# atenpas/agile_grasp

Measured on AMD Instinct MI355X. Metric: grasp hypotheses/sec on 300k-pt cloud @2000 samples, higher is better.
Workload: dtype f64

## Files before the change

agile_grasp_amd/binding.py:

```python
from __future__ import annotations

import ctypes as C
import os

import numpy as np

_HERE = os.path.dirname(os.path.abspath(__file__))
_LIB = None

NORMALS_DETERMINISTIC = 0
NORMALS_RAND50 = 1


class AghParams(C.Structure):
    _fields_ = [
        ("finger_width", C.c_double),
        ("hand_outer_diameter", C.c_double),
        ("hand_depth", C.c_double),
        ("hand_height", C.c_double),
        ("init_bite", C.c_double),
        ("nn_radius_taubin", C.c_double),
        ("nn_radius_hands", C.c_double),
        ("nn_radius_normals", C.c_double),
        ("cam_origin", (C.c_double * 3) * 2),
# ... 21 lines not shown
        ("cam_source", "<i4"),
        ("n_in_box", "<i4"),
        ("half_antipodal", "u1"),
        ("full_antipodal", "u1"),
        ("svm_keep", "u1"),
        ("valid", "u1"),
        ("finger_index", "<i4"),
        ("depth_index", "<i4"),
        ("epoch", "<i4"),
    ]
)
FRAME_DTYPE = np.dtype(
    [
        ("sample", "<f8", 3),
        ("normal", "<f8", 3),
        ("axis", "<f8", 3),
        ("binormal", "<f8", 3),
        ("params", "<f8", 10),
        ("eigenvalue", "<f8"),
        ("n_nb", "<i4"),
        ("majority_cam", "<i4"),
        ("max_index", "<i4"),
        ("valid", "<i4"),
    ]
)
HANDLE_DTYPE = np.dtype([("axis", "<f8", 3), ("center", "<f8", 3), ("approach", "<f8", 3), ("binormal", "<f8", 3),
                         ("hands_center", "<f8", 3), ("width", "<f8"), ("n_inliers", "<i4"), ("first_inlier", "<i4")])
assert HYP_DTYPE.itemsize == 160 and FRAME_DTYPE.itemsize == 200 and HANDLE_DTYPE.itemsize == 136

EXPORTS = [
    "agh_default_params", "agh_create", "agh_destroy", "agh_last_error", "agh_set_cloud", "agh_set_cloud_device", "agh_set_cloud_batch", "agh_set_cloud_batch_device",
    "agh_preprocess", "agh_preprocess_device", "agh_localize", "agh_localize_device", "agh_localize_begin", "agh_localize_stage", "agh_localize_end", "agh_get_cloud", "agh_find_handles", "agh_find_hands", "agh_find_hands_device", "agh_load_svm", "agh_load_svm_file", "agh_classify",
    "agh_classify_device", "agh_get_frames", "agh_get_neighbor_counts", "agh_get_images", "agh_get_hog",
    "agh_get_normals", "agh_get_timing", "agh_get_timing_counts", "agh_set_profile", "agh_synchronize", "agh_selftest_math",
    "agh_set_training_images", "agh_get_training_images", "agh_hog_images", "agh_train_svm", "agh_save_svm_file",
    "agh_load_svm_model", "agh_get_learning_points", "agh_get_epoch", "agh_get_packed_images", "agh_classify_images", "agh_comm_rccl_origin",
    "agh_save_svm_file_ex", "agh_comm_unique_id", "agh_comm_init", "agh_comm_init_local", "agh_comm_destroy", "agh_comm_rank", "agh_comm_last_count", "agh_comm_last_exchange", "agh_comm_set_segment_records", "agh_comm_inject_fault",
    "agh_shard_slice", "agh_find_hands_sharded_device", "agh_find_hands_sharded", "agh_classify_sharded_device",
    "agh_classify_sharded", "agh_default_plane_params", "agh_remove_plane", "agh_get_plane_inliers",
    "agh_get_plane_candidates", "agh_plane_replay",
]


def comm_unique_id() -> bytes:
    buf = (C.c_uint8 * 128)()
    rc = load_library().agh_comm_unique_id(buf)
    if rc != 0:
        raise AghError(rc, "agh_comm_unique_id failed (is RCCL installed?)")
    return bytes(buf)


def comm_init_local(contexts) -> None:
    arr = (C.c_void_p * len(contexts))(*[c._h for c in contexts])
    rc = load_library().agh_comm_init_local(arr, C.c_int32(len(contexts)))
    if rc != 0:
        raise AghError(rc, "agh_comm_init_local failed")


def shard_slice(n: int, rank: int, n_ranks: int):
    lo, hi = C.c_int64(0), C.c_int64(0)
    load_library().agh_shard_slice(C.c_int64(n), C.c_int32(rank), C.c_int32(n_ranks), C.byref(lo), C.byref(hi))
    return lo.value, hi.value


def comm_rccl_origin() -> str:
    lib = load_library()
    lib.agh_comm_rccl_origin.restype = C.c_char_p
# ... 498 lines not shown
        return out[:n].copy(), keep[:n].copy()

    def find_hands_sharded_torch(self, samples_t, out_t, nout_t, calculates_antipodal: bool = False, stream=None):
        S = samples_t.shape[0]
        cap = out_t.numel() // 160
        r, g = self.comm_rank()
        lo, hi = shard_slice(S, r, g)
        self.last_samples = hi - lo
        self._check(self.lib.agh_find_hands_sharded_device(
            self._h, C.c_void_p(samples_t.data_ptr()), C.c_int64(S), C.c_int(1 if calculates_antipodal else 0),
            C.c_void_p(out_t.data_ptr()), C.c_int64(cap), C.c_void_p(nout_t.data_ptr()),
            C.c_void_p(stream) if stream else None))

    def classify_sharded_torch(self, keep_t=None, stream=None):
        self._check(self.lib.agh_classify_sharded_device(
            self._h, C.c_void_p(keep_t.data_ptr()) if keep_t is not None else None, C.c_void_p(stream) if stream else None))

    def hog(self):
        desc = np.zeros((max(self.last_n, 1), 3528), np.float32)
        sums = np.zeros(max(self.last_n, 1), np.float64)
        n = self._check(self.lib.agh_get_hog(self._h, _p(desc, C.c_float), _p(sums, C.c_double), C.c_int64(self.last_n)))
        return desc[:n], sums[:n]

    def timing(self, counts: bool = False):
        t = AghTiming()
        self._check(self.lib.agh_get_timing(self._h, C.byref(t)))
        ms = {t.name[i].decode(): float(t.ms[i]) for i in range(t.n)}
        if counts:
            cnt = (C.c_int32 * 16)()
            self._check(self.lib.agh_get_timing_counts(self._h, cnt, C.c_int32(16)))
            return ms, {t.name[i].decode(): int(cnt[i]) for i in range(t.n)}
        return ms

    def set_profile(self, level: int):
        self._check(self.lib.agh_set_profile(self._h, C.c_int32(level)))

    def synchronize(self):
        self._check(self.lib.agh_synchronize(self._h))

    def selftest_math(self, n: int = 1 << 20, seed: int = 1) -> int:
        return int(self.lib.agh_selftest_math(self._h, C.c_int64(n), C.c_uint64(seed)))

    def set_cloud_torch(self, xyz_t, cam_t, stream=None):
        assert xyz_t.is_cuda and xyz_t.is_contiguous()
        self._keep = [xyz_t, cam_t]
        self.n = xyz_t.shape[0]
        self._check(self.lib.agh_set_cloud_device(
            self._h, C.c_void_p(xyz_t.data_ptr()), C.c_int64(xyz_t.stride(0) * 4),
            C.c_void_p(cam_t.data_ptr()) if cam_t is not None else None, C.c_int64(self.n),
            C.c_void_p(stream) if stream else None))

    def find_hands_torch(self, samples_t, out_t, nout_t, calculates_antipodal: bool = False, stream=None):
        S = samples_t.shape[0]
        cap = out_t.numel() // 160
        self.last_samples = S
        self._check(self.lib.agh_find_hands_device(
            self._h, C.c_void_p(samples_t.data_ptr()), C.c_int64(S), C.c_int(1 if calculates_antipodal else 0),
            C.c_void_p(out_t.data_ptr()), C.c_int64(cap), C.c_void_p(nout_t.data_ptr()),
            C.c_void_p(stream) if stream else None))

    def classify_torch(self, keep_t=None, stream=None):
        self._check(self.lib.agh_classify_device(self._h, C.c_void_p(keep_t.data_ptr()) if keep_t is not None else None,
                                                 C.c_void_p(stream) if stream else None))
```

agile_grasp_amd/csrc/agh_internal.h:

```cpp
#pragma once

#include <hip/hip_runtime.h>
#include <stdint.h>

#include <string>
#include <vector>

#include "agh.h"

namespace agh
{

constexpr int kBboxBlocks = 128;
constexpr int kCellCap = 1 << 21;
constexpr int kCellStride = kCellCap + 4;
constexpr int kMaxRows = 128;
constexpr int kNumSums = 37;
constexpr int kSumStride = 40;
constexpr int kSlots = 8;
constexpr int kImageWords = 250;
constexpr int kBigListGrid = 512;
constexpr int kSweepWg4MinSamples = 4096;
constexpr int64_t kNormalsChunk = 16384;

struct GridDesc
{
  double mn[3];
  double cell;
  double inv_cell;
  int dim[3];
  int ncell;
  unsigned done;
  unsigned ticket;
};

constexpr int kMaxClouds = 64;
struct GridView
{
  const GridDesc* desc;
  const int* cell_start;
  const float4* sorted;
  const int* cloud_off;
  int n_clouds;
};

struct HandGeom
{
  double finger_width, hand_outer_diameter, hand_depth, hand_height, init_bite;
  double cam_origin[2][3];
  double cos_a[8], sin_a[8];
  double fs[20];
  double thr[40];
  int n_thr;
  int lo_idx[20], hi_idx[20];
  double depths[16];
  double backs[16];
  double boxy[16];
  int n_depths;
  double cos_antipodal;
  double xlut_lo, xlut_scale;
  double ylut_lo, ylut_scale;
  unsigned char xlut[1024];
  unsigned char ylut[64];
  int x_probes, y_probes;
};
// ... 110 lines not shown
  float* d_vox_xyz = nullptr;
  int32_t* d_vox_cam = nullptr;
  int64_t vox_cap = 0;
  float* d_raw_xyz = nullptr;
  float* d_stage_xyz = nullptr;
  int64_t stage_cap = 0;
  hipStream_t stage_stream = nullptr;
  hipEvent_t stage_done = nullptr;
  LocalizeState loc;
  int64_t raw_cap = 0;
  PlaneState* plane = nullptr;

  agh_hypothesis* d_h_hands = nullptr;
  unsigned long long* d_h_bits = nullptr;
  int* d_h_rowcnt = nullptr;
  int* d_h_first = nullptr;
  int* d_h_n = nullptr;
  int* d_h_idx = nullptr;
  int* d_h_counts = nullptr;
  int* d_h_tmp = nullptr;
  agh_handle* d_h_handles = nullptr;
  int64_t h_cap = 0;

  int n_clouds = 1;
  int clouds_cap = 0;
  std::vector<int64_t> cloud_off;
  std::vector<int32_t> cloud_off_i32;
  bool cloud_off_on_device = false;
  bool defer_cloud_count = false;
  bool n_is_bound = false;
  int* d_cloud_off = nullptr;
  int32_t* d_scloud = nullptr;
  GridDesc* d_desc = nullptr;
  float* d_bbox_part = nullptr;
  int* d_cell_start = nullptr;
  int* d_cell_count = nullptr;
  int* d_block_sums = nullptr;
  unsigned long long* d_tile_state = nullptr;
  unsigned build_gen = 0;
  bool grid_clean = false;
  int* d_cell_of = nullptr;
  int* d_rank_of = nullptr;
  float4* d_sorted = nullptr;
  int64_t grid_cap = 0;
  bool has_cloud = false;
  const int32_t* pending_cam_host = nullptr;
  int64_t pending_cam_n = 0;
  bool cloud_async = false;

  int64_t s_cap = 0;
  int32_t* d_samples = nullptr;
  double* d_sums = nullptr;
  int32_t* d_nt = nullptr;
  int32_t* d_ovf = nullptr;
  int32_t* d_nh = nullptr;
  int32_t* d_status = nullptr;
  int* d_weight = nullptr;
  uint8_t* d_vmask = nullptr;
  int* d_order = nullptr;
  int* d_order_sweep = nullptr;
  int order_frame_s = 0;
  const int32_t* order_frame_samples = nullptr;
  int order_sweep_s = 0;
  const int32_t* order_sweep_samples = nullptr;
  float4* d_nbr = nullptr;
  int64_t nbr_stride = 0;
  double* d_eig = nullptr;
// ... 278 lines not shown
{
  int begin[kMaxRows];
  int prefix[kMaxRows + 1];
  int seg_row[64];
  int nrows;
  int total;
  int bad;
};

constexpr double kSlabMargin = 1e-6;
template <bool SLAB = false>
__device__ __forceinline__ void build_rows(const GridView& gv, float qx, float qy, float qz, double rpad, RowTable& rt,
  const double* slab_axis = nullptr, double slab_hh = 0.0, const GridDesc* gpre = nullptr)
{
  const GridDesc& g = gpre ? *gpre : *gv.desc;
  const int tid = threadIdx.x;
  const int lx = cell_coord(g, (double) qx - rpad, 0), hx = cell_coord(g, (double) qx + rpad, 0);
  const int ly = cell_coord(g, (double) qy - rpad, 1), hy = cell_coord(g, (double) qy + rpad, 1);
  const int lz = cell_coord(g, (double) qz - rpad, 2), hz = cell_coord(g, (double) qz + rpad, 2);
  const int ny = hy - ly + 1, nz = hz - lz + 1;
  const int nrows = ny * nz;
  if (tid == 0)
  {
    rt.nrows = nrows;
    rt.bad = nrows > kMaxRows;
  }
  if (nrows <= kMaxRows)
  {
    for (int t = tid; t < nrows; t += blockDim.x)
    {
      const int tq = (int) (((float) t + 0.5f) * (1.0f / (float) ny));
      const int cy = ly + (t - tq * ny), cz = lz + tq;
      const double y0 = g.mn[1] + cy * g.cell, z0 = g.mn[2] + cz * g.cell;
      const double dy = fmax(fmax(y0 - (double) qy, (double) qy - (y0 + g.cell)), 0.0);
      const double dz = fmax(fmax(z0 - (double) qz, (double) qz - (z0 + g.cell)), 0.0);
      int b = 0, len = 0;
      const double rem = rpad * rpad - (dy * dy + dz * dz);
      if (rem >= 0.0)
      {
        const double xr = sqrt(rem);
        double xlo = (double) qx - xr, xhi = (double) qx + xr;
        bool keep = true;
        if (SLAB)
        {
          const double ya = (y0 - kSlabMargin) - (double) qy, yb = (y0 + g.cell + kSlabMargin) - (double) qy;
          const double za = (z0 - kSlabMargin) - (double) qz, zb = (z0 + g.cell + kSlabMargin) - (double) qz;
          const double ey0 = slab_axis[1] * ya, ey1 = slab_axis[1] * yb, ez0 = slab_axis[2] * za, ez1 = slab_axis[2] * zb;
          const double L = fmin(ey0, ey1) + fmin(ez0, ez1), U = fmax(ey0, ey1) + fmax(ez0, ez1);
          const double lo_n = (-1.0 * (slab_hh + kSlabMargin)) - U, hi_n = (slab_hh + kSlabMargin) - L;
          const double ax = slab_axis[0];
          if (fabs(ax) > 1e-9)
          {
            const double inv_ax = 1.0 / ax;
            const double b1 = lo_n * inv_ax, b2 = hi_n * inv_ax;
            xlo = fmax(xlo, ((double) qx + fmin(b1, b2)) - kSlabMargin);
            xhi = fmin(xhi, ((double) qx + fmax(b1, b2)) + kSlabMargin);
            keep = xlo <= xhi;
          }
          else
            keep = (lo_n < 0.0) & (hi_n > 0.0);
          keep = keep | !(L == L && U == U);
        }
        if (keep)
        {
          const int lxr = max(lx, cell_coord(g, xlo, 0)), hxr = min(hx, cell_coord(g, xhi, 0));
          const int base = (cz * g.dim[1] + cy) * g.dim[0];
          b = gv.cell_start[base + lxr];
          len = hxr >= lxr ? gv.cell_start[base + hxr + 1] - b : 0;
        }
      }
      rt.begin[t] = b;
      rt.prefix[t + 1] = len;
    }
  }
  __syncthreads();
  if (tid < 64)
// ... 197 lines not shown
```

agile_grasp_amd/csrc/api.hip:

```cpp
#include "agh_internal.h"

#include <algorithm>
#include <atomic>
#include <cmath>
#include <cstdio>
#include <cstdlib>
#include <cstring>

using namespace agh;


namespace
{
thread_local std::string g_create_error;
std::atomic<int32_t> g_epoch{ 0 };
}

namespace agh
{
int32_t next_epoch()
{
  int32_t e;
  do
    e = (int32_t) ((uint32_t) g_epoch.fetch_add(1) + 1u) & 0x7fffffff;
// ... 201 lines not shown
  return AGH_OK;
}

constexpr int64_t kMirrorMaxRecords = 1 << 16;
static inline int64_t pin_round(int64_t b) { return (b + 255) & ~(int64_t) 255; }
int ensure_host_staging(Ctx* c, int64_t samples, int64_t records)
{
  if (c->h_pin && samples <= c->h_pin_samples && records <= c->h_pin_records)
    return AGH_OK;
  const int64_t ns = std::max<int64_t>(std::max<int64_t>(samples, c->h_pin_samples), 1024);
  const int64_t nr = std::max<int64_t>(std::max<int64_t>(records, c->h_pin_records), 1024);
  if (c->h_pin)
  {
    HIPCHK(c, hipStreamSynchronize(c->stream));
    (void) hipHostFree(c->h_pin);
    c->h_pin = nullptr;
    c->h_pin_samples = c->h_pin_records = 0;
  }
  void* p = nullptr;
  HIPCHK(c, hipHostMalloc(&p, (size_t) (kPinHeaderBytes + pin_round(ns * 4) + nr * (int64_t) sizeof(agh_hypothesis)), hipHostMallocDefault));
  c->h_pin = static_cast<uint8_t*>(p);
  c->h_pin_samples = ns;
  c->h_pin_records = nr;
  return AGH_OK;
}

int ensure_clouds(Ctx* c, int C)
{
  if (C <= c->clouds_cap)
    return AGH_OK;
  int rc;
  if ((rc = dev_alloc(c, &c->d_desc, (size_t) C)) || (rc = dev_alloc(c, &c->d_cell_start, (size_t) C * (size_t) kCellStride)) ||
      (rc = dev_alloc(c, &c->d_cell_count, (size_t) C * kCellCap)) || (rc = dev_alloc(c, &c->d_bbox_part, (size_t) C * kBboxBlocks * 6)) ||
      (rc = dev_alloc(c, &c->d_tile_state, (size_t) C * (kCellCap / 1024))))
    return rc;
  c->clouds_cap = C;
  c->grid_clean = false;
  return AGH_OK;
}

int ensure_draws(Ctx* c, int64_t count, hipStream_t st)
{
  if (count <= c->draws_cap)
    return AGH_OK;
  std::vector<int32_t> h((size_t) count);
  GlibcRand g(c->p.rand_seed);
  for (int64_t i = 0; i < count; i++)
    h[i] = g.next();
  int rc;
  if ((rc = dev_alloc(c, &c->d_draws, (size_t) count)))
    return rc;
  HIPCHK(c, hipMemcpyAsync(c->d_draws, h.data(), sizeof(int32_t) * count, hipMemcpyHostToDevice, st));
  HIPCHK(c, hipStreamSynchronize(st));
  c->draws_cap = count;
  return AGH_OK;
}

__global__ void k_iota(int32_t* out, int base, int n)
{
  const int i = blockIdx.x * blockDim.x + threadIdx.x;
  if (i < n)
    out[i] = base + i;
}

int normals_pass(Ctx* c, int64_t p0, int64_t p1, hipStream_t st)
{
  for (int64_t b0 = p0; b0 < p1; b0 += kNormalsChunk)
// ... 107 lines not shown
  *out = nullptr;
  int ndev = 0;
  if (hipGetDeviceCount(&ndev) != hipSuccess || ndev <= 0)
  {
    g_create_error = "no HIP device is visible (this library has no CPU path)";
    return AGH_ERR_NO_DEVICE;
  }
  if (p->device < 0 || p->device >= ndev)
  {
    g_create_error = "device ordinal out of range";
    return AGH_ERR_INVALID_ARGUMENT;
  }
  hipDeviceProp_t prop;
  if (hipGetDeviceProperties(&prop, p->device) != hipSuccess)
  {
    g_create_error = "hipGetDeviceProperties failed";
    return AGH_ERR_HIP;
  }
  if (std::strncmp(prop.gcnArchName, "gfx950", 6) != 0)
  {
    g_create_error = std::string("device is ") + prop.gcnArchName + ", this build targets gfx950 (MI355X) only";
    return AGH_ERR_NO_DEVICE;
  }
  if (!(p->finger_width > 0) || !(p->hand_outer_diameter > p->finger_width) || !(p->hand_depth > 0) ||
      !(p->nn_radius_taubin > 0) || !(p->nn_radius_hands > 0) || !(p->nn_radius_normals > 0))
  {
    g_create_error = "invalid hand geometry or radii";
    return AGH_ERR_INVALID_ARGUMENT;
  }
  agh_ctx* ctx = new agh_ctx();
  Ctx* c = &ctx->c;
  c->p = *p;
  c->device = p->device;
#ifdef AGH_DEBUG_HOOKS
  if (const char* e = std::getenv("AGH_DEBUG_STOP_SWEEP"))
    c->debug_stop_sweep = std::atoi(e);
  if (const char* e = std::getenv("AGH_DEBUG_STOP_MOMENTS"))
    c->debug_stop_moments = std::atoi(e);
  if (const char* e = std::getenv("AGH_DEBUG_STOP_FRAME"))
    c->debug_stop_frame = std::atoi(e);
  if (const char* e = std::getenv("AGH_DEBUG_STOP_HOG"))
    c->debug_stop_hog = std::atoi(e);
#endif
  std::string gerr;
  build_geometry(*p, &c->geom, &gerr);
  if (!gerr.empty())
  {
    g_create_error = gerr;
    delete ctx;
    return AGH_ERR_INVALID_ARGUMENT;
  }
  auto fail = [&](int rc) {
    g_create_error = c->err;
    agh_destroy(ctx);
    return rc;
  };
  if (hipSetDevice(c->device) != hipSuccess || hipStreamCreate(&c->stream) != hipSuccess)
  {
    c->err = "hipSetDevice/hipStreamCreate failed";
    return fail(AGH_ERR_HIP);
  }
  int rc;
  if ((rc = ensure_clouds(c, 1)) || (rc = dev_alloc(c, &c->d_cloud_off, (size_t) kMaxClouds + 1)) ||
      (rc = dev_alloc(c, &c->d_block_sums, 4096)) ||
      (rc = dev_alloc(c, &c->d_flags, 8)) || (rc = dev_alloc(c, &c->d_nout, 1)) ||
      (rc = dev_alloc(c, &c->d_geom, 1)) || (rc = dev_alloc(c, &c->d_hog, 1)) ||
      (rc = dev_alloc(c, &c->d_svm_w, 3528)))
    return fail(rc);
  HogTablesDev* ht = new HogTablesDev();
  hog_tables_host(ht);
  hipError_t e1 = hipMemcpy(c->d_hog, ht, sizeof(HogTablesDev), hipMemcpyHostToDevice);
  delete ht;
  hipError_t e2 = hipMemcpy(c->d_geom, &c->geom, sizeof(HandGeom), hipMemcpyHostToDevice);
  hipError_t e3 = hipMemset(c->d_flags, 0, 8 * sizeof(int32_t));
  if (e1 != hipSuccess || e2 != hipSuccess || e3 != hipSuccess)
  {
    c->err = "uploading tables failed";
    return fail(AGH_ERR_HIP);
  }
  *out = ctx;
  return AGH_OK;
}

void agh_destroy(agh_ctx* ctx)
{
  if (!ctx)
    return;
  Ctx* c = &ctx->c;
  (void) hipSetDevice(c->device);
  if (c->stream)
    (void) hipStreamSynchronize(c->stream);
  comm_release(c);
  plane_release(c);
  void* ptrs[] = { c->own_xyz, c->own_cam, c->d_desc, c->d_bbox_part, c->d_cell_start, c->d_cell_count, c->d_block_sums, c->d_cell_of,
    c->d_rank_of, c->d_sorted, c->d_samples, c->d_sums, c->d_nt, c->d_nh, c->d_status, c->d_nbr, c->d_eig, c->d_frames, c->d_slots,
    c->d_images, c->d_slot_index, c->d_scan_tmp, c->d_out_own, c->d_nout, c->d_out_images, c->d_draw_ofs, c->d_draws,
    c->d_flags, c->d_normals, c->d_svm_w, c->d_hog, c->d_geom, c->d_desc_out, c->d_svm_sums, c->d_keep, c->d_vox_desc,
    c->d_weight, c->d_order, c->d_order_sweep, c->d_vmask, c->d_cloud_off, c->d_scloud, c->d_idx_own, c->d_tile_state, c->d_h_hands, c->d_h_bits, c->d_h_rowcnt, c->d_h_first,
    c->d_h_n, c->d_h_idx, c->d_h_counts, c->d_h_handles, c->d_h_tmp, c->d_images_cam, c->d_xbuf, c->d_nbuf, c->d_xcnt, c->d_cls_images, c->d_cls_keep, c->d_cls_sums, c->d_dbg, c->d_svm_svT, c->d_svm_alpha, c->d_cls_desc, c->d_cls_kbuf, c->d_vox_code, c->d_vox_blk, c->d_vox_blk2, c->d_vox_total, c->d_vox_bitmap, c->d_vox_xyz, c->d_vox_cam, c->d_raw_xyz, c->d_huge_stage, c->d_huge_key, c->d_huge_count, c->d_huge_sorted, c->d_huge_normals, c->d_huge_base, c->d_stage_xyz, c->d_ovf };
  for (void* p : ptrs)
    if (p)
      (void) hipFree(p);
  if (c->h_pin)
    (void) hipHostFree(c->h_pin);
  if (c->h_pin_handles)
    (void) hipHostFree(c->h_pin_handles);
  if (c->h_pin_keep)
    (void) hipHostFree(c->h_pin_keep);
  if (c->h_vox_desc)
    (void) hipHostFree(c->h_vox_desc);
  for (hipEvent_t e : c->ev)
    (void) hipEventDestroy(e);
  if (c->copy_done)
    (void) hipEventDestroy(c->copy_done);
  if (c->copy_gate)
    (void) hipEventDestroy(c->copy_gate);
  if (c->xyz_copied)
    (void) hipEventDestroy(c->xyz_copied);
  if (c->copy_stream)
    (void) hipStreamDestroy(c->copy_stream);
  if (c->stage_done)
    (void) hipEventDestroy(c->stage_done);
  if (c->stage_stream)
    (void) hipStreamDestroy(c->stage_stream);
  if (c->stream)
    (void) hipStreamDestroy(c->stream);
  delete ctx;
}

namespace
{
struct CloudOffArg
// ... 905 lines not shown
    float ms = 0.f;
    if (hipEventElapsedTime(&ms, c->ev[i - 1], c->ev[i]) != hipSuccess)
      ms = 0.f;
    int slot = -1;
    for (int j = 0; j < k; j++)
      if (std::strcmp(out->name[j], c->ev_name[i]) == 0)
        slot = j;
    if (slot < 0)
    {
      if (k >= AGH_TIMING_SLOTS)
        continue;
      slot = k++;
      out->name[slot] = c->ev_name[i];
    }
    out->ms[slot] += ms;
    c->timing_counts[slot]++;
    out->total_ms += ms;
  }
  out->n = k;
  c->ev_used = 0;
  c->ev_name.clear();
  return AGH_OK;
}

int agh_get_timing_counts(agh_ctx* ctx, int32_t* counts, int32_t cap)
{
  if (!ctx || !counts || cap < 0)
    return AGH_ERR_INVALID_ARGUMENT;
  for (int i = 0; i < cap && i < AGH_TIMING_SLOTS; i++)
    counts[i] = ctx->c.timing_counts[i];
  return AGH_OK;
}

int64_t agh_selftest_math(agh_ctx* ctx, int64_t n, uint64_t seed)
{
  if (!ctx)
    return AGH_ERR_INVALID_ARGUMENT;
  return selftest_math(&ctx->c, n, seed);
}

}
```

agile_grasp_amd/csrc/grid.hip:

```cpp
#include "agh_internal.h"

#include <algorithm>
#include <cstdlib>

namespace agh
{

__global__ void k_desc_reset(GridDesc* d)
{
  d += blockIdx.x;
  d->done = 0u;
  d->ticket = 0u;
}

__device__ void desc_finish(GridDesc* d, double base_cell, int64_t n, const float lo[3], const float hi[3])
{
  double mn[3], mx[3];
  for (int a = 0; a < 3; a++)
  {
    const bool any = n > 0 && lo[a] <= hi[a];
    mn[a] = any ? (double) lo[a] : 0.0;
    mx[a] = any ? (double) hi[a] : 0.0;
  }
  double cell = base_cell;
  int dim[3];
  for (;;)
  {
    double prod = 1.0;
    for (int a = 0; a < 3; a++)
    {
      dim[a] = (int) floor((mx[a] - mn[a]) / cell) + 1;
      prod *= (double) dim[a];
    }
    if (prod <= (double) kCellCap)
      break;
    cell *= 2.0;
  }
  for (int a = 0; a < 3; a++)
  {
    d->mn[a] = mn[a];
    d->dim[a] = dim[a];
  }
  d->cell = cell;
  d->inv_cell = 1.0 / cell;
// ... 20 lines not shown
      mn[a] = fminf(mn[a], fminf(pf ? pv[a] : INFINITY, qf ? qv[a] : INFINITY));
      mx[a] = fmaxf(mx[a], fmaxf(pf ? pv[a] : -INFINITY, qf ? qv[a] : -INFINITY));
    }
  }
  constexpr int kW = kBboxThreads / 64;
  __shared__ float smn[kW][3], smx[kW][3];
  for (int a = 0; a < 3; a++)
    for (int o = 32; o > 0; o >>= 1)
    {
      mn[a] = fminf(mn[a], __shfl_down(mn[a], o));
      mx[a] = fmaxf(mx[a], __shfl_down(mx[a], o));
    }
  if ((threadIdx.x & 63) == 0)
    for (int a = 0; a < 3; a++)
    {
      smn[threadIdx.x >> 6][a] = mn[a];
      smx[threadIdx.x >> 6][a] = mx[a];
    }
  __syncthreads();
  if (threadIdx.x < 3)
  {
    const int a = threadIdx.x;
    float lo = smn[0][a], hi = smx[0][a];
    for (int w = 1; w < kW; w++)
    {
      lo = fminf(lo, smn[w][a]);
      hi = fmaxf(hi, smx[w][a]);
    }
    part[blockIdx.x * 6 + a] = lo;
    part[blockIdx.x * 6 + 3 + a] = hi;
  }
}

__device__ __forceinline__ void desc_from_parts(const float* __restrict__ part, int nparts, double base_cell, int64_t n, GridDesc* g)
{
  __shared__ float red[4][6];
  const int tid = threadIdx.x, lane = tid & 63;
  float lo[3] = { INFINITY, INFINITY, INFINITY }, hi[3] = { -INFINITY, -INFINITY, -INFINITY };
  for (int b = tid; b < nparts; b += blockDim.x)
    for (int a = 0; a < 3; a++)
    {
      lo[a] = fminf(lo[a], part[b * 6 + a]);
      hi[a] = fmaxf(hi[a], part[b * 6 + 3 + a]);
    }
  for (int a = 0; a < 3; a++)
    for (int o = 32; o > 0; o >>= 1)
    {
      lo[a] = fminf(lo[a], __shfl_xor(lo[a], o));
      hi[a] = fmaxf(hi[a], __shfl_xor(hi[a], o));
    }
  if (lane == 0 && tid < 256)
    for (int a = 0; a < 3; a++)
    {
      red[tid >> 6][a] = lo[a];
      red[tid >> 6][3 + a] = hi[a];
    }
  __syncthreads();
  if (tid == 0)
  {
    for (int a = 0; a < 3; a++)
      for (int w = 1; w < 4; w++)
      {
        lo[a] = fminf(lo[a], red[w][a]);
        hi[a] = fmaxf(hi[a], red[w][3 + a]);
      }
    desc_finish(g, base_cell, n, lo, hi);
  }
  __syncthreads();
}

__global__ __launch_bounds__(256) void k_cell_count(const float* __restrict__ xyz, int64_t stride,
  const int* __restrict__ cloud_off, GridDesc* __restrict__ d, int* __restrict__ cell_of, int* __restrict__ rank_of,
  int* __restrict__ count, const float* __restrict__ part, int nparts, double base_cell)
{
  const int64_t p0 = cloud_off[blockIdx.y], n = cloud_off[blockIdx.y + 1] - p0;
  xyz += p0 * stride;
  cell_of += p0;
  rank_of += p0;
  count += (int64_t) blockIdx.y * kCellCap;
  __shared__ GridDesc gs;
  desc_from_parts(part + (int64_t) blockIdx.y * kBboxBlocks * 6, nparts, base_cell, n, &gs);
  const GridDesc g = gs;
  if (blockIdx.x == 0 && threadIdx.x == 0)
  {
    GridDesc* o = d + blockIdx.y;
    for (int a = 0; a < 3; a++)
    {
      o->mn[a] = g.mn[a];
      o->dim[a] = g.dim[a];
    }
    o->cell = g.cell;
    o->inv_cell = g.inv_cell;
    o->ncell = g.ncell;
  }
  const int lane = threadIdx.x & 63;
  const int64_t step = (int64_t) gridDim.x * blockDim.x;
  const int64_t n_up = (n + 63) & ~(int64_t) 63;
  for (int64_t i = blockIdx.x * (int64_t) blockDim.x + threadIdx.x; i < n_up; i += step)
  {
    int c = -1;
    if (i < n)
    {
      const float* p = xyz + i * stride;
      const int cx = cell_coord(g, (double) p[0], 0), cy = cell_coord(g, (double) p[1], 1),
                cz = cell_coord(g, (double) p[2], 2);
      c = (cz * g.dim[1] + cy) * g.dim[0] + cx;
      if (!(isfinite(p[0]) && isfinite(p[1]) && isfinite(p[2])))
        c = (int) (i % (int64_t) g.ncell);
    }
    const int prev = __shfl_up(c, 1);
    const bool head = (lane == 0) || (c != prev);
    const unsigned long long hm = __ballot(head);
    const int hl = 63 - __clzll((long long) (hm & ((2ull << lane) - 1ull)));
    const unsigned long long after = (hl == 63) ? 0ull : (hm >> (hl + 1));
    const int runlen = after ? (__ffsll((long long) after)) : (64 - hl);
    int base = 0;
    if (head && c >= 0)
      base = atomicAdd(&count[c], runlen);
    base = __shfl(base, hl);
    if (i < n)
    {
      cell_of[i] = c;
      rank_of[i] = base + (lane - hl);
    }
  }
}

constexpr int kScanBlock = 4096;

__device__ __forceinline__ int block_scan_excl(int v, int* total)
{
  __shared__ int wsum[4];
  const int lane = threadIdx.x & 63, w = threadIdx.x >> 6;
  const int inc = wave_incl_scan_i32(v);
  if (lane == 63)
    wsum[w] = inc;
  __syncthreads();
  int base = 0;
  for (int k = 0; k < w; k++)
    base += wsum[k];
  *total = wsum[0] + wsum[1] + wsum[2] + wsum[3];
  __syncthreads();
  return base + inc - v;
}

__global__ __launch_bounds__(256) void k_cell_scan(int* __restrict__ count, GridDesc* __restrict__ d,
  unsigned long long* __restrict__ tile_state, unsigned gen, int* __restrict__ cell_start, const int* __restrict__ cloud_off)
{
  __shared__ int s_prefix;
  const int p0 = cloud_off[blockIdx.y], n = cloud_off[blockIdx.y + 1] - p0;
  count += (int64_t) blockIdx.y * kCellCap;
  tile_state += (int64_t) blockIdx.y * (kCellCap / kScanBlock);
  cell_start += (int64_t) blockIdx.y * kCellStride;
  d += blockIdx.y;
  const int ncell = d->ncell;
  for (int tile = blockIdx.x; tile * kScanBlock < ncell; tile += gridDim.x)
  {
  const int b0 = tile * kScanBlock;
  int4 v[4];
  int sum = 0;
  for (int k = 0; k < 4; k++)
  {
    v[k] = reinterpret_cast<const int4*>(count + b0)[threadIdx.x * 4 + k];
    sum += (v[k].x + v[k].y) + (v[k].z + v[k].w);
  }
  int total;
  int ex = block_scan_excl(sum, &total);
  const unsigned long long tag = (unsigned long long) gen << 34;
  if (threadIdx.x < 64)
  {
    const int lane = threadIdx.x;
    int prefix = 0;
    if (lane == 0)
      __hip_atomic_store(&tile_state[tile], tag | ((tile == 0 ? 2ull : 1ull) << 32) | (unsigned) total, __ATOMIC_RELEASE,
        __HIP_MEMORY_SCOPE_AGENT);
    for (int j0 = tile - 1; j0 >= 0; j0 -= 64)
    {
      const int j = j0 - lane;
      unsigned long long w = 0;
      for (;;)
// ... 12 lines not shown
      const int stop = incl ? __ffsll((long long) incl) - 1 : 63;
      int val = (j >= 0 && lane <= stop) ? (int) (unsigned) w : 0;
      for (int o = 32; o > 0; o >>= 1)
        val += __shfl_xor(val, o);
      prefix += val;
      if (incl)
        break;
    }
    if (lane == 0)
    {
      if (tile != 0)
        __hip_atomic_store(&tile_state[tile], tag | (2ull << 32) | (unsigned) (prefix + total), __ATOMIC_RELEASE,
          __HIP_MEMORY_SCOPE_AGENT);
      s_prefix = prefix;
    }
  }
  __syncthreads();
  ex += s_prefix + p0;
  for (int k = 0; k < 4; k++)
  {
    int4 o;
    o.x = ex;
    o.y = o.x + v[k].x;
    o.z = o.y + v[k].y;
    o.w = o.z + v[k].z;
    ex = o.w + v[k].w;
    reinterpret_cast<int4*>(cell_start + b0)[threadIdx.x * 4 + k] = o;
    reinterpret_cast<int4*>(count + b0)[threadIdx.x * 4 + k] = make_int4(0, 0, 0, 0);
  }
  if (tile == 0 && threadIdx.x == 0)
    cell_start[ncell] = p0 + n;
  __syncthreads();
  }
}

__global__ __launch_bounds__(256) void k_scatter(const float* __restrict__ xyz, int64_t stride,
  const int32_t* __restrict__ cam, const int* __restrict__ cloud_off, const int* __restrict__ cell_of,
  const int* __restrict__ rank_of, const int* __restrict__ cell_start, float4* __restrict__ sorted)
{
  const int64_t p0 = cloud_off[blockIdx.y], p1 = cloud_off[blockIdx.y + 1];
  cell_start += (int64_t) blockIdx.y * kCellStride;
  for (int64_t i = p0 + blockIdx.x * (int64_t) blockDim.x + threadIdx.x; i < p1; i += (int64_t) gridDim.x * blockDim.x)
  {
    const int pos = cell_start[cell_of[i]] + rank_of[i];
    const float* p = xyz + i * stride;
    const unsigned w = ((unsigned) i << 1) | (cam ? (unsigned) (cam[i] & 1) : 0u);
    sorted[pos] = make_float4(p[0], p[1], p[2], __uint_as_float(w));
  }
}

int grid_build(Ctx* c, hipStream_t st)
{
  const int C = c->n_clouds;
  int64_t nmax = 0;
  for (int k = 0; k < C; k++)
    nmax = std::max<int64_t>(nmax, c->cloud_off[(size_t) k + 1] - c->cloud_off[(size_t) k]);
  const int nblk = (int) std::max<int64_t>(1, std::min<int64_t>((nmax + 255) / 256, 2048));
  if (!c->grid_clean)
  {
    hipMemsetAsync(c->d_cell_count, 0, sizeof(int) * (size_t) kCellCap * c->clouds_cap, st);
    hipMemsetAsync(c->d_tile_state, 0, sizeof(unsigned long long) * (size_t) (kCellCap / kScanBlock) * c->clouds_cap, st);
    hipLaunchKernelGGL(k_desc_reset, dim3(c->clouds_cap), dim3(1), 0, st, c->d_desc);
    c->build_gen = 0;
  }
  c->grid_clean = false;
  if (++c->build_gen >= (1u << 30))
  {
    hipMemsetAsync(c->d_tile_state, 0, sizeof(unsigned long long) * (size_t) (kCellCap / kScanBlock) * c->clouds_cap, st);
    c->build_gen = 1;
  }
  bool cam_gate = false;
  if (c->pending_cam_host)
  {
    if (!c->copy_stream && !c->copy_stream_failed &&
        (hipStreamCreateWithFlags(&c->copy_stream, hipStreamNonBlocking) != hipSuccess ||
         hipEventCreateWithFlags(&c->copy_done, hipEventDisableTiming) != hipSuccess ||
         hipEventCreateWithFlags(&c->copy_gate, hipEventDisableTiming) != hipSuccess))
    {
      if (c->copy_gate)
        (void) hipEventDestroy(c->copy_gate);
      if (c->copy_done)
        (void) hipEventDestroy(c->copy_done);
      if (c->copy_stream)
        (void) hipStreamDestroy(c->copy_stream);
      c->copy_gate = nullptr;
      c->copy_done = nullptr;
      c->copy_stream = nullptr;
      c->copy_stream_failed = true;
    }
    if (c->copy_stream)
      cam_gate = hipEventRecord(c->copy_gate, st) == hipSuccess && hipStreamWaitEvent(c->copy_stream, c->copy_gate, 0) == hipSuccess;
  }
  const double base_cell = std::max(0.02, c->p.nn_radius_hands / 4.0);
  const int nparts = std::max(1, std::min(nblk, kBboxBlocks));
  hipLaunchKernelGGL(k_bbox, dim3(nparts, C), dim3(kBboxThreads), 0, st, c->d_xyz, c->stride_floats,
    (const int*) c->d_cloud_off, c->d_bbox_part);
  hipLaunchKernelGGL(k_cell_count, dim3(nblk, C), dim3(256), 0, st, c->d_xyz, c->stride_floats, (const int*) c->d_cloud_off,
    c->d_desc, c->d_cell_of, c->d_rank_of, c->d_cell_count, (const float*) c->d_bbox_part, nparts, base_cell);
  hipLaunchKernelGGL(k_cell_scan, dim3(C == 1 ? 256 : 64, C), dim3(256), 0, st, c->d_cell_count, c->d_desc, c->d_tile_state,
    c->build_gen, c->d_cell_start, (const int*) c->d_cloud_off);
  if (c->pending_cam_host)
  {
    hipStream_t cs = (c->copy_stream && cam_gate) ? c->copy_stream : st;
    hipError_t e = hipMemcpyAsync(c->own_cam, c->pending_cam_host, sizeof(int32_t) * (size_t) c->pending_cam_n,
      hipMemcpyHostToDevice, cs);
    c->pending_cam_host = nullptr;
    c->cam_copy_on_copy_stream = cs != st;
    if (e == hipSuccess && cs != st)
    {
      e = hipEventRecord(c->copy_done, cs);
      if (e == hipSuccess)
        e = hipStreamWaitEvent(st, c->copy_done, 0);
    }
    if (e != hipSuccess)
      return AGH_ERR_HIP;
  }
  if (nmax > 0)
    hipLaunchKernelGGL(k_scatter, dim3(nblk, C), dim3(256), 0, st, c->d_xyz, c->stride_floats, c->d_cam,
      (const int*) c->d_cloud_off, c->d_cell_of, c->d_rank_of, c->d_cell_start, c->d_sorted);
  if (hipGetLastError() != hipSuccess)
    return AGH_ERR_HIP;
  c->grid_clean = true;
  return AGH_OK;
}

}
```

include/agh.h:

```cpp
#ifndef AGH_H
#define AGH_H

#include <stdint.h>

#ifdef __cplusplus
extern "C" {
#endif

#define AGH_VERSION 1

typedef enum agh_status
{
  AGH_OK = 0,
  AGH_ERR_INVALID_ARGUMENT = -1,
  AGH_ERR_NO_DEVICE = -2,
  AGH_ERR_HIP = -3,
  AGH_ERR_CAPACITY = -4,
  AGH_ERR_NO_CLOUD = -5,
  AGH_ERR_NO_SVM = -6,
  AGH_ERR_IO = -7,
  AGH_ERR_STATE = -8,
  AGH_ERR_RETRY = -9
} agh_status;

// ... 175 lines not shown
int agh_save_svm_file_ex(const char* path, int32_t kernel_type, const float* sv, int32_t n_sv, int32_t n_weights,
  const double* alpha, double rho, double C, int32_t max_iter, double eps);
int agh_load_svm_model(agh_ctx* ctx, int32_t kernel_type, const float* sv, int32_t n_sv, int32_t n_weights,
  const double* alpha, double rho);

#define AGH_COMM_ID_BYTES 128
int agh_comm_unique_id(uint8_t id[AGH_COMM_ID_BYTES]);
int agh_comm_init(agh_ctx* ctx, int32_t rank, int32_t n_ranks, const uint8_t id[AGH_COMM_ID_BYTES]);
int agh_comm_init_local(agh_ctx* const* ctxs, int32_t n_ranks);
int agh_comm_destroy(agh_ctx* ctx);
int agh_comm_rank(const agh_ctx* ctx, int32_t* rank, int32_t* n_ranks);
const char* agh_comm_rccl_origin(void);
int agh_comm_last_count(const agh_ctx* ctx, int64_t* n_hyp);
int agh_comm_last_exchange(const agh_ctx* ctx, int64_t* segment_bytes, int32_t* n_ranks, int32_t* via_rccl);
int agh_comm_inject_fault(agh_ctx* ctx, int32_t sites);

int agh_comm_set_segment_records(agh_ctx* ctx, int64_t records);
void agh_shard_slice(int64_t n, int32_t rank, int32_t n_ranks, int64_t* lo, int64_t* hi);
int agh_find_hands_sharded_device(agh_ctx* ctx, const int32_t* d_sample_idx, int64_t n_samples, int calculates_antipodal,
  agh_hypothesis* d_out, int64_t cap, int64_t* d_n_out, void* hip_stream);
int agh_find_hands_sharded(agh_ctx* ctx, const int32_t* sample_idx, int64_t n_samples, int calculates_antipodal,
  agh_hypothesis* out, int64_t cap, int64_t* n_out);
int agh_classify_sharded_device(agh_ctx* ctx, uint8_t* d_keep, void* hip_stream);
int agh_classify_sharded(agh_ctx* ctx, agh_hypothesis* out, uint8_t* keep, int64_t cap, int64_t* n_kept);

int agh_get_frames(agh_ctx* ctx, agh_frame* out, int64_t cap);
int agh_get_neighbor_counts(agh_ctx* ctx, int32_t* n_taubin, int32_t* n_hands, int64_t cap);
int agh_get_images(agh_ctx* ctx, uint8_t* images, int64_t cap_hyp);
int agh_get_hog(agh_ctx* ctx, float* desc, double* sums, int64_t cap_hyp);
int agh_get_normals(agh_ctx* ctx, double* normals, int64_t cap_points);
int agh_get_learning_points(agh_ctx* ctx, int64_t hyp, double* points, int32_t* cam_source, int64_t cap, int64_t* n_out);
int agh_get_timing(agh_ctx* ctx, agh_timing* out);
int agh_get_timing_counts(agh_ctx* ctx, int32_t* counts, int32_t cap);
int agh_set_profile(agh_ctx* ctx, int32_t level);
int agh_synchronize(agh_ctx* ctx);
int64_t agh_selftest_math(agh_ctx* ctx, int64_t n, uint64_t seed);

#ifdef __cplusplus
}
#endif
#endif
```

Measured before the change: 4.091 million.

## Reuse previous grid descriptor with margin to skip bbox pass on warm builds

```diff
diff --git a/agile_grasp_amd/binding.py b/agile_grasp_amd/binding.py
--- a/agile_grasp_amd/binding.py
+++ b/agile_grasp_amd/binding.py
@@ -77,7 +77,7 @@
     "agh_default_params", "agh_create", "agh_destroy", "agh_last_error", "agh_set_cloud", "agh_set_cloud_device", "agh_set_cloud_batch", "agh_set_cloud_batch_device",
     "agh_preprocess", "agh_preprocess_device", "agh_localize", "agh_localize_device", "agh_localize_begin", "agh_localize_stage", "agh_localize_end", "agh_get_cloud", "agh_find_handles", "agh_find_hands", "agh_find_hands_device", "agh_load_svm", "agh_load_svm_file", "agh_classify",
     "agh_classify_device", "agh_get_frames", "agh_get_neighbor_counts", "agh_get_images", "agh_get_hog",
-    "agh_get_normals", "agh_get_timing", "agh_get_timing_counts", "agh_set_profile", "agh_synchronize", "agh_selftest_math",
+    "agh_get_normals", "agh_get_timing", "agh_get_timing_counts", "agh_get_grid_stats", "agh_set_profile", "agh_synchronize", "agh_selftest_math",
     "agh_set_training_images", "agh_get_training_images", "agh_hog_images", "agh_train_svm", "agh_save_svm_file",
     "agh_load_svm_model", "agh_get_learning_points", "agh_get_epoch", "agh_get_packed_images", "agh_classify_images", "agh_comm_rccl_origin",
     "agh_save_svm_file_ex", "agh_comm_unique_id", "agh_comm_init", "agh_comm_init_local", "agh_comm_destroy", "agh_comm_rank", "agh_comm_last_count", "agh_comm_last_exchange", "agh_comm_set_segment_records", "agh_comm_inject_fault",
@@ -642,6 +642,11 @@
             return ms, {t.name[i].decode(): int(cnt[i]) for i in range(t.n)}
         return ms
 
+    def grid_stats(self) -> dict:
+        v = (C.c_int64 * 3)()
+        self._check(self.lib.agh_get_grid_stats(self._h, v, C.c_int32(3)))
+        return {"builds": int(v[0]), "cold": int(v[1]), "misses": int(v[2])}
+
     def set_profile(self, level: int):
         self._check(self.lib.agh_set_profile(self._h, C.c_int32(level)))
 
diff --git a/agile_grasp_amd/csrc/agh_internal.h b/agile_grasp_amd/csrc/agh_internal.h
--- a/agile_grasp_amd/csrc/agh_internal.h
+++ b/agile_grasp_amd/csrc/agh_internal.h
@@ -12,6 +12,8 @@
 {
 
 constexpr int kBboxBlocks = 128;
+constexpr int kCountBlocks = 2048;
+constexpr int kGridMargin = 2;
 constexpr int kCellCap = 1 << 21;
 constexpr int kCellStride = kCellCap + 4;
 constexpr int kMaxRows = 128;
@@ -30,7 +32,7 @@
   double inv_cell;
   int dim[3];
   int ncell;
-  unsigned done;
+  unsigned open;
   unsigned ticket;
 };
 
@@ -207,7 +209,14 @@
   int* d_cloud_off = nullptr;
   int32_t* d_scloud = nullptr;
   GridDesc* d_desc = nullptr;
+  GridDesc* d_desc_next = nullptr;
   float* d_bbox_part = nullptr;
+  float* d_count_part = nullptr;
+  unsigned* d_grid_miss = nullptr;
+  bool grid_miss_zeroed = false;
+  bool grid_force_cold = false;
+  int grid_key_clouds = 0;
+  int64_t grid_builds = 0, grid_cold_builds = 0;
   int* d_cell_start = nullptr;
   int* d_cell_count = nullptr;
   int* d_block_sums = nullptr;
@@ -552,8 +561,20 @@
       const int tq = (int) (((float) t + 0.5f) * (1.0f / (float) ny));
       const int cy = ly + (t - tq * ny), cz = lz + tq;
       const double y0 = g.mn[1] + cy * g.cell, z0 = g.mn[2] + cz * g.cell;
-      const double dy = fmax(fmax(y0 - (double) qy, (double) qy - (y0 + g.cell)), 0.0);
-      const double dz = fmax(fmax(z0 - (double) qz, (double) qz - (z0 + g.cell)), 0.0);
+      double ylo = y0, yhi = y0 + g.cell, zlo = z0, zhi = z0 + g.cell;
+      bool open_row = false;
+      if (g.open)
+      {
+        const bool oy0 = cy == 0 && (g.open & 4u), oy1 = cy == g.dim[1] - 1 && (g.open & 8u);
+        const bool oz0 = cz == 0 && (g.open & 16u), oz1 = cz == g.dim[2] - 1 && (g.open & 32u);
+        ylo = oy0 ? -INFINITY : ylo;
+        yhi = oy1 ? INFINITY : yhi;
+        zlo = oz0 ? -INFINITY : zlo;
+        zhi = oz1 ? INFINITY : zhi;
+        open_row = oy0 | oy1 | oz0 | oz1;
+      }
+      const double dy = fmax(fmax(ylo - (double) qy, (double) qy - yhi), 0.0);
+      const double dz = fmax(fmax(zlo - (double) qz, (double) qz - zhi), 0.0);
       int b = 0, len = 0;
       const double rem = rpad * rpad - (dy * dy + dz * dz);
       if (rem >= 0.0)
@@ -561,7 +582,7 @@
         const double xr = sqrt(rem);
         double xlo = (double) qx - xr, xhi = (double) qx + xr;
         bool keep = true;
-        if (SLAB)
+        if (SLAB && !open_row)
         {
           const double ya = (y0 - kSlabMargin) - (double) qy, yb = (y0 + g.cell + kSlabMargin) - (double) qy;
           const double za = (z0 - kSlabMargin) - (double) qz, zb = (z0 + g.cell + kSlabMargin) - (double) qz;
diff --git a/agile_grasp_amd/csrc/api.hip b/agile_grasp_amd/csrc/api.hip
--- a/agile_grasp_amd/csrc/api.hip
+++ b/agile_grasp_amd/csrc/api.hip
@@ -257,7 +257,10 @@
   int rc;
   if ((rc = dev_alloc(c, &c->d_desc, (size_t) C)) || (rc = dev_alloc(c, &c->d_cell_start, (size_t) C * (size_t) kCellStride)) ||
       (rc = dev_alloc(c, &c->d_cell_count, (size_t) C * kCellCap)) || (rc = dev_alloc(c, &c->d_bbox_part, (size_t) C * kBboxBlocks * 6)) ||
-      (rc = dev_alloc(c, &c->d_tile_state, (size_t) C * (kCellCap / 1024))))
+      (rc = dev_alloc(c, &c->d_tile_state, (size_t) C * (kCellCap / 1024))) || (rc = dev_alloc(c, &c->d_desc_next, (size_t) C)) ||
+      (rc = dev_alloc(c, &c->d_count_part, (size_t) C * kCountBlocks * 6)))
+    return rc;
+  if (!c->d_grid_miss && (rc = dev_alloc(c, &c->d_grid_miss, 1)))
     return rc;
   c->clouds_cap = C;
   c->grid_clean = false;
@@ -431,6 +434,8 @@
   Ctx* c = &ctx->c;
   c->p = *p;
   c->device = p->device;
+  if (const char* e = std::getenv("AGH_GRID_COLD"))
+    c->grid_force_cold = std::atoi(e) != 0;
 #ifdef AGH_DEBUG_HOOKS
   if (const char* e = std::getenv("AGH_DEBUG_STOP_SWEEP"))
     c->debug_stop_sweep = std::atoi(e);
@@ -496,7 +501,8 @@
     c->d_images, c->d_slot_index, c->d_scan_tmp, c->d_out_own, c->d_nout, c->d_out_images, c->d_draw_ofs, c->d_draws,
     c->d_flags, c->d_normals, c->d_svm_w, c->d_hog, c->d_geom, c->d_desc_out, c->d_svm_sums, c->d_keep, c->d_vox_desc,
     c->d_weight, c->d_order, c->d_order_sweep, c->d_vmask, c->d_cloud_off, c->d_scloud, c->d_idx_own, c->d_tile_state, c->d_h_hands, c->d_h_bits, c->d_h_rowcnt, c->d_h_first,
-    c->d_h_n, c->d_h_idx, c->d_h_counts, c->d_h_handles, c->d_h_tmp, c->d_images_cam, c->d_xbuf, c->d_nbuf, c->d_xcnt, c->d_cls_images, c->d_cls_keep, c->d_cls_sums, c->d_dbg, c->d_svm_svT, c->d_svm_alpha, c->d_cls_desc, c->d_cls_kbuf, c->d_vox_code, c->d_vox_blk, c->d_vox_blk2, c->d_vox_total, c->d_vox_bitmap, c->d_vox_xyz, c->d_vox_cam, c->d_raw_xyz, c->d_huge_stage, c->d_huge_key, c->d_huge_count, c->d_huge_sorted, c->d_huge_normals, c->d_huge_base, c->d_stage_xyz, c->d_ovf };
+    c->d_h_n, c->d_h_idx, c->d_h_counts, c->d_h_handles, c->d_h_tmp, c->d_images_cam, c->d_xbuf, c->d_nbuf, c->d_xcnt, c->d_cls_images, c->d_cls_keep, c->d_cls_sums, c->d_dbg, c->d_svm_svT, c->d_svm_alpha, c->d_cls_desc, c->d_cls_kbuf, c->d_vox_code, c->d_vox_blk, c->d_vox_blk2, c->d_vox_total, c->d_vox_bitmap, c->d_vox_xyz, c->d_vox_cam, c->d_raw_xyz, c->d_huge_stage, c->d_huge_key, c->d_huge_count, c->d_huge_sorted, c->d_huge_normals, c->d_huge_base, c->d_stage_xyz, c->d_ovf,
+    c->d_desc_next, c->d_count_part, c->d_grid_miss };
   for (void* p : ptrs)
     if (p)
       (void) hipFree(p);
@@ -1468,6 +1474,25 @@
   return AGH_OK;
 }
 
+int agh_get_grid_stats(agh_ctx* ctx, int64_t* stats, int32_t cap)
+{
+  if (!ctx || (!stats && cap > 0) || cap < 0)
+    return AGH_ERR_INVALID_ARGUMENT;
+  Ctx* c = &ctx->c;
+  unsigned miss = 0;
+  HIPCHK(c, hipSetDevice(c->device));
+  if (c->d_grid_miss && c->grid_miss_zeroed)
+  {
+    HIPCHK(c, hipDeviceSynchronize());
+    HIPCHK(c, hipMemcpy(&miss, c->d_grid_miss, sizeof(unsigned), hipMemcpyDeviceToHost));
+  }
+  const int64_t v[3] = { c->grid_builds, c->grid_cold_builds, (int64_t) miss };
+  int k = 0;
+  for (; k < cap && k < 3; k++)
+    stats[k] = v[k];
+  return k;
+}
+
 int64_t agh_selftest_math(agh_ctx* ctx, int64_t n, uint64_t seed)
 {
   if (!ctx)
diff --git a/agile_grasp_amd/csrc/grid.hip b/agile_grasp_amd/csrc/grid.hip
--- a/agile_grasp_amd/csrc/grid.hip
+++ b/agile_grasp_amd/csrc/grid.hip
@@ -9,7 +9,7 @@
 __global__ void k_desc_reset(GridDesc* d)
 {
   d += blockIdx.x;
-  d->done = 0u;
+  d->open = 0u;
   d->ticket = 0u;
 }
 
@@ -96,23 +96,48 @@
   }
 }
 
-__device__ __forceinline__ void desc_from_parts(const float* __restrict__ part, int nparts, double base_cell, int64_t n, GridDesc* g)
+static_assert(kCountBlocks % 256 == 0, "reduce_parts: whole rounds of 256 slots");
+
+__device__ __forceinline__ void wave_minmax3(float lo[3], float hi[3])
+{
+  for (int a = 0; a < 3; a++)
+  {
+    lo[a] = fminf(lo[a], __int_as_float(xor_partner_i32<32>(__float_as_int(lo[a]))));
+    hi[a] = fmaxf(hi[a], __int_as_float(xor_partner_i32<32>(__float_as_int(hi[a]))));
+    lo[a] = fminf(lo[a], __int_as_float(xor_partner_i32<16>(__float_as_int(lo[a]))));
+    hi[a] = fmaxf(hi[a], __int_as_float(xor_partner_i32<16>(__float_as_int(hi[a]))));
+    lo[a] = fminf(lo[a], __int_as_float(xor_partner_i32<8>(__float_as_int(lo[a]))));
+    hi[a] = fmaxf(hi[a], __int_as_float(xor_partner_i32<8>(__float_as_int(hi[a]))));
+    lo[a] = fminf(lo[a], __int_as_float(xor_partner_i32<4>(__float_as_int(lo[a]))));
+    hi[a] = fmaxf(hi[a], __int_as_float(xor_partner_i32<4>(__float_as_int(hi[a]))));
+    lo[a] = fminf(lo[a], __int_as_float(xor_partner_i32<2>(__float_as_int(lo[a]))));
+    hi[a] = fmaxf(hi[a], __int_as_float(xor_partner_i32<2>(__float_as_int(hi[a]))));
+    lo[a] = fminf(lo[a], __int_as_float(xor_partner_i32<1>(__float_as_int(lo[a]))));
+    hi[a] = fmaxf(hi[a], __int_as_float(xor_partner_i32<1>(__float_as_int(hi[a]))));
+  }
+}
+
+__device__ __forceinline__ void reduce_parts(const float* __restrict__ part, int nparts, float lo[3], float hi[3])
 {
   __shared__ float red[4][6];
   const int tid = threadIdx.x, lane = tid & 63;
-  float lo[3] = { INFINITY, INFINITY, INFINITY }, hi[3] = { -INFINITY, -INFINITY, -INFINITY };
-  for (int b = tid; b < nparts; b += blockDim.x)
-    for (int a = 0; a < 3; a++)
-    {
-      lo[a] = fminf(lo[a], part[b * 6 + a]);
-      hi[a] = fmaxf(hi[a], part[b * 6 + 3 + a]);
-    }
   for (int a = 0; a < 3; a++)
-    for (int o = 32; o > 0; o >>= 1)
-    {
-      lo[a] = fminf(lo[a], __shfl_xor(lo[a], o));
-      hi[a] = fmaxf(hi[a], __shfl_xor(hi[a], o));
-    }
+  {
+    lo[a] = INFINITY;
+    hi[a] = -INFINITY;
+  }
+#pragma unroll
+  for (int k = 0; k < kCountBlocks / 256; k++)
+  {
+    const int b = tid + 256 * k;
+    if (b < nparts)
+      for (int a = 0; a < 3; a++)
+      {
+        lo[a] = fminf(lo[a], part[b * 6 + a]);
+        hi[a] = fmaxf(hi[a], part[b * 6 + 3 + a]);
+      }
+  }
+  wave_minmax3(lo, hi);
   if (lane == 0 && tid < 256)
     for (int a = 0; a < 3; a++)
     {
@@ -121,30 +146,43 @@
     }
   __syncthreads();
   if (tid == 0)
-  {
     for (int a = 0; a < 3; a++)
       for (int w = 1; w < 4; w++)
       {
         lo[a] = fminf(lo[a], red[w][a]);
         hi[a] = fmaxf(hi[a], red[w][3 + a]);
       }
+}
+
+__device__ __forceinline__ void desc_from_parts(const float* __restrict__ part, int nparts, double base_cell, int64_t n, GridDesc* g)
+{
+  float lo[3], hi[3];
+  reduce_parts(part, nparts, lo, hi);
+  if (threadIdx.x == 0)
     desc_finish(g, base_cell, n, lo, hi);
-  }
-  __syncthreads();
-}
-
+  __syncthreads();
+}
+
+template <bool COLD>
 __global__ __launch_bounds__(256) void k_cell_count(const float* __restrict__ xyz, int64_t stride,
-  const int* __restrict__ cloud_off, GridDesc* __restrict__ d, int* __restrict__ cell_of, int* __restrict__ rank_of,
-  int* __restrict__ count, const float* __restrict__ part, int nparts, double base_cell)
+  const int* __restrict__ cloud_off, GridDesc* __restrict__ d, const GridDesc* __restrict__ kept, int* __restrict__ cell_of,
+  int* __restrict__ rank_of, int* __restrict__ count, const float* __restrict__ part, int nparts, double base_cell,
+  float* __restrict__ part_out)
 {
   const int64_t p0 = cloud_off[blockIdx.y], n = cloud_off[blockIdx.y + 1] - p0;
   xyz += p0 * stride;
   cell_of += p0;
   rank_of += p0;
   count += (int64_t) blockIdx.y * kCellCap;
-  __shared__ GridDesc gs;
-  desc_from_parts(part + (int64_t) blockIdx.y * kBboxBlocks * 6, nparts, base_cell, n, &gs);
-  const GridDesc g = gs;
+  GridDesc g;
+  if (COLD)
+  {
+    __shared__ GridDesc gs;
+    desc_from_parts(part + (int64_t) blockIdx.y * kBboxBlocks * 6, nparts, base_cell, n, &gs);
+    g = gs;
+  }
+  else
+    g = kept[blockIdx.y];
   if (blockIdx.x == 0 && threadIdx.x == 0)
   {
     GridDesc* o = d + blockIdx.y;
@@ -156,7 +194,9 @@
     o->cell = g.cell;
     o->inv_cell = g.inv_cell;
     o->ncell = g.ncell;
-  }
+    o->open = 0u;
+  }
+  float mn[3] = { INFINITY, INFINITY, INFINITY }, mx[3] = { -INFINITY, -INFINITY, -INFINITY };
   const int lane = threadIdx.x & 63;
   const int64_t step = (int64_t) gridDim.x * blockDim.x;
   const int64_t n_up = (n + 63) & ~(int64_t) 63;
@@ -166,11 +206,20 @@
     if (i < n)
     {
       const float* p = xyz + i * stride;
-      const int cx = cell_coord(g, (double) p[0], 0), cy = cell_coord(g, (double) p[1], 1),
-                cz = cell_coord(g, (double) p[2], 2);
+      const float px = p[0], py = p[1], pz = p[2];
+      const int cx = cell_coord(g, (double) px, 0), cy = cell_coord(g, (double) py, 1), cz = cell_coord(g, (double) pz, 2);
       c = (cz * g.dim[1] + cy) * g.dim[0] + cx;
-      if (!(isfinite(p[0]) && isfinite(p[1]) && isfinite(p[2])))
+      if (!(isfinite(px) && isfinite(py) && isfinite(pz)))
         c = (int) (i % (int64_t) g.ncell);
+      else
+      {
+        mn[0] = fminf(mn[0], px);
+        mn[1] = fminf(mn[1], py);
+        mn[2] = fminf(mn[2], pz);
+        mx[0] = fmaxf(mx[0], px);
+        mx[1] = fmaxf(mx[1], py);
+        mx[2] = fmaxf(mx[2], pz);
+      }
     }
     const int prev = __shfl_up(c, 1);
     const bool head = (lane == 0) || (c != prev);
@@ -188,6 +237,65 @@
       rank_of[i] = base + (lane - hl);
     }
   }
+  __shared__ float smn[4][3], smx[4][3];
+  wave_minmax3(mn, mx);
+  if (lane == 0)
+    for (int a = 0; a < 3; a++)
+    {
+      smn[threadIdx.x >> 6][a] = mn[a];
+      smx[threadIdx.x >> 6][a] = mx[a];
+    }
+  __syncthreads();
+  if (threadIdx.x < 3)
+  {
+    const int a = threadIdx.x;
+    const float lo = fminf(fminf(smn[0][a], smn[1][a]), fminf(smn[2][a], smn[3][a]));
+    const float hi = fmaxf(fmaxf(smx[0][a], smx[1][a]), fmaxf(smx[2][a], smx[3][a]));
+    float* slot = part_out + ((int64_t) blockIdx.y * kCountBlocks + blockIdx.x) * 6;
+    slot[a] = lo;
+    slot[3 + a] = hi;
+  }
+}
+
+__device__ void desc_next(const GridDesc u, GridDesc* used, GridDesc* next, unsigned* miss, double base_cell, int64_t n,
+  const float lo[3], const float hi[3], bool cold)
+{
+  GridDesc t;
+  desc_finish(&t, base_cell, n, lo, hi);
+  const bool any = n > 0 && lo[0] <= hi[0];
+  unsigned open = 0u;
+  bool fits = !cold && any && u.cell == t.cell;
+  if (any)
+    for (int a = 0; a < 3; a++)
+    {
+      if (floor(((double) lo[a] - u.mn[a]) * u.inv_cell) < 0.0)
+        open |= 1u << (2 * a);
+      if (floor(((double) hi[a] - u.mn[a]) * u.inv_cell) > (double) (u.dim[a] - 1))
+        open |= 2u << (2 * a);
+      fits = fits && u.dim[a] - t.dim[a] <= 4 * kGridMargin;
+    }
+  if (open)
+  {
+    used->open = open;
+    atomicAdd(miss, 1u);
+  }
+  GridDesc o = u;
+  if (!fits || open)
+  {
+    int m = kGridMargin;
+    if ((double) (t.dim[0] + 2 * m) * (double) (t.dim[1] + 2 * m) * (double) (t.dim[2] + 2 * m) > (double) kCellCap)
+      m = 0;
+    o = t;
+    for (int a = 0; a < 3; a++)
+    {
+      o.mn[a] = t.mn[a] - m * t.cell;
+      o.dim[a] = t.dim[a] + 2 * m;
+    }
+    o.ncell = o.dim[0] * o.dim[1] * o.dim[2];
+  }
+  o.open = 0u;
+  o.ticket = 0u;
+  *next = o;
 }
 
 constexpr int kScanBlock = 4096;
@@ -209,7 +317,8 @@
 }
 
 __global__ __launch_bounds__(256) void k_cell_scan(int* __restrict__ count, GridDesc* __restrict__ d,
-  unsigned long long* __restrict__ tile_state, unsigned gen, int* __restrict__ cell_start, const int* __restrict__ cloud_off)
+  unsigned long long* __restrict__ tile_state, unsigned gen, int* __restrict__ cell_start, const int* __restrict__ cloud_off,
+  const float* __restrict__ part, int nparts, GridDesc* __restrict__ next, unsigned* __restrict__ miss, double base_cell, int cold)
 {
   __shared__ int s_prefix;
   const int p0 = cloud_off[blockIdx.y], n = cloud_off[blockIdx.y + 1] - p0;
@@ -288,6 +397,13 @@
     cell_start[ncell] = p0 + n;
   __syncthreads();
   }
+  if (blockIdx.x == gridDim.x - 1)
+  {
+    float lo[3], hi[3];
+    reduce_parts(part + (int64_t) blockIdx.y * kCountBlocks * 6, nparts, lo, hi);
+    if (threadIdx.x == 0)
+      desc_next(*d, d, next + blockIdx.y, miss, base_cell, n, lo, hi, cold != 0);
+  }
 }
 
 __global__ __launch_bounds__(256) void k_scatter(const float* __restrict__ xyz, int64_t stride,
@@ -311,7 +427,13 @@
   int64_t nmax = 0;
   for (int k = 0; k < C; k++)
     nmax = std::max<int64_t>(nmax, c->cloud_off[(size_t) k + 1] - c->cloud_off[(size_t) k]);
-  const int nblk = (int) std::max<int64_t>(1, std::min<int64_t>((nmax + 255) / 256, 2048));
+  const int nblk = (int) std::max<int64_t>(1, std::min<int64_t>((nmax + 255) / 256, kCountBlocks));
+  const bool cold = !c->grid_clean || c->grid_force_cold || c->grid_key_clouds != C;
+  if (!c->grid_miss_zeroed)
+  {
+    hipMemsetAsync(c->d_grid_miss, 0, sizeof(unsigned), st);
+    c->grid_miss_zeroed = true;
+  }
   if (!c->grid_clean)
   {
     hipMemsetAsync(c->d_cell_count, 0, sizeof(int) * (size_t) kCellCap * c->clouds_cap, st);
@@ -348,13 +470,24 @@
       cam_gate = hipEventRecord(c->copy_gate, st) == hipSuccess && hipStreamWaitEvent(c->copy_stream, c->copy_gate, 0) == hipSuccess;
   }
   const double base_cell = std::max(0.02, c->p.nn_radius_hands / 4.0);
-  const int nparts = std::max(1, std::min(nblk, kBboxBlocks));
-  hipLaunchKernelGGL(k_bbox, dim3(nparts, C), dim3(kBboxThreads), 0, st, c->d_xyz, c->stride_floats,
-    (const int*) c->d_cloud_off, c->d_bbox_part);
-  hipLaunchKernelGGL(k_cell_count, dim3(nblk, C), dim3(256), 0, st, c->d_xyz, c->stride_floats, (const int*) c->d_cloud_off,
-    c->d_desc, c->d_cell_of, c->d_rank_of, c->d_cell_count, (const float*) c->d_bbox_part, nparts, base_cell);
+  if (cold)
+  {
+    const int nparts = std::max(1, std::min(nblk, kBboxBlocks));
+    hipLaunchKernelGGL(k_bbox, dim3(nparts, C), dim3(kBboxThreads), 0, st, c->d_xyz, c->stride_floats,
+      (const int*) c->d_cloud_off, c->d_bbox_part);
+    hipLaunchKernelGGL(k_cell_count<true>, dim3(nblk, C), dim3(256), 0, st, c->d_xyz, c->stride_floats, (const int*) c->d_cloud_off,
+      c->d_desc, (const GridDesc*) c->d_desc_next, c->d_cell_of, c->d_rank_of, c->d_cell_count, (const float*) c->d_bbox_part,
+      nparts, base_cell, c->d_count_part);
+  }
+  else
+    hipLaunchKernelGGL(k_cell_count<false>, dim3(nblk, C), dim3(256), 0, st, c->d_xyz, c->stride_floats, (const int*) c->d_cloud_off,
+      c->d_desc, (const GridDesc*) c->d_desc_next, c->d_cell_of, c->d_rank_of, c->d_cell_count, (const float*) nullptr, 0,
+      base_cell, c->d_count_part);
   hipLaunchKernelGGL(k_cell_scan, dim3(C == 1 ? 256 : 64, C), dim3(256), 0, st, c->d_cell_count, c->d_desc, c->d_tile_state,
-    c->build_gen, c->d_cell_start, (const int*) c->d_cloud_off);
+    c->build_gen, c->d_cell_start, (const int*) c->d_cloud_off, (const float*) c->d_count_part, nblk, c->d_desc_next,
+    c->d_grid_miss, base_cell, cold ? 1 : 0);
+  c->grid_builds++;
+  c->grid_cold_builds += cold ? 1 : 0;
   if (c->pending_cam_host)
   {
     hipStream_t cs = (c->copy_stream && cam_gate) ? c->copy_stream : st;
@@ -377,6 +510,7 @@
   if (hipGetLastError() != hipSuccess)
     return AGH_ERR_HIP;
   c->grid_clean = true;
+  c->grid_key_clouds = C;
   return AGH_OK;
 }
 
diff --git a/include/agh.h b/include/agh.h
--- a/include/agh.h
+++ b/include/agh.h
@@ -231,6 +231,7 @@
 int agh_get_learning_points(agh_ctx* ctx, int64_t hyp, double* points, int32_t* cam_source, int64_t cap, int64_t* n_out);
 int agh_get_timing(agh_ctx* ctx, agh_timing* out);
 int agh_get_timing_counts(agh_ctx* ctx, int32_t* counts, int32_t cap);
+int agh_get_grid_stats(agh_ctx* ctx, int64_t* stats, int32_t cap);
 int agh_set_profile(agh_ctx* ctx, int32_t level);
 int agh_synchronize(agh_ctx* ctx);
 int64_t agh_selftest_math(agh_ctx* ctx, int64_t n, uint64_t seed);
```

Measured after the change: 4.212 million (median of 6 runs). 1.03x the previous value.
